# vovach777/llcomp

Hardware: AMD Instinct MI355X
Metric: encode+decode MPix/s on 4K RGB8, bit-exact (higher is better)
Workload: dtype int32

## Files before the change

### llcomp_amd/csrc/dec_rows_asm.hpp

```cpp
#pragma once
#include <cstdint>

namespace llcomp_mi {

#define LD_E0L "v32"
#define LD_E0H "v33"
#define LD_E0 "v[32:33]"
#define LD_E5L "v34"
#define LD_E5H "v35"
#define LD_E5 "v[34:35]"
#define LD_E6L "v36"
#define LD_E6H "v37"
#define LD_E6 "v[36:37]"
#define LD_E7L "v38"
#define LD_E7H "v39"
#define LD_E7 "v[38:39]"
#define LD_E1L "v40"
#define LD_E1H "v41"
#define LD_E1 "v[40:41]"
#define LD_E2L "v42"
#define LD_E2H "v43"
#define LD_E2 "v[42:43]"
#define LD_E3L "v44"
#define LD_E3H "v45"
#define LD_E3 "v[44:45]"
#define LD_E4L "v48"
#define LD_E4H "v49"
#define LD_E4 "v[48:49]"
#define LD_WINL "v46"
#define LD_WIN "v[46:47]"
#define LD_PROD "v50"
#define LD_R1 "v51"
#define LD_DIFF "v52"
#define LD_OFF "v52"
#define LD_EX "v32"
#define LD_W "v33"
#define LD_RUN "v40"
#define LD_NX "v41"
#define LD_T "v42"
#define LD_SX "s[56:57]"
#define LD_SA "s[58:59]"
#define LD_SW "s[60:61]"
#define LD_SP "s[62:63]"
#define LD_S5 "s[64:65]"
#define LD_SU "s[66:67]"
#define LD_SD "s[68:69]"
#define LD_S1L "s[68:69]"
#define LD_SM "s[70:71]"
#define LD_S1 "s70"
#define LD_S2 "s71"

#define LD_SPLIT(EL)                                                                                                       \
    "v_mul_u32_u24_sdwa " LD_PROD ", " EL ", %[range] dst_sel:DWORD dst_unused:UNUSED_PAD src0_sel:BYTE_1 src1_sel:DWORD\n\t" \
    "v_lshrrev_b32_e32 " LD_R1 ", 8, " LD_PROD "\n\t"                                                                      \
    "v_sub_u32_e32 %[range], %[range], " LD_R1 "\n\t"
#define LD_REFILL(N)                                         \
    "v_cmp_gt_u32_e32 vcc, %[c100], %[range]\n\t"            \
    "s_and_saveexec_b64 " LD_SW ", vcc\n\t"                  \
    "s_cbranch_execz .Lrf" N "_%=\n\t"                       \
    "v_lshlrev_b32_e32 %[range], 8, %[range]\n\t"            \
    "v_perm_b32 %[low], %[low], %[w32], %[sel]\n\t"          \
    "v_lshrrev_b32_e32 %[w32], 8, %[w32]\n"                   \
    ".Lrf" N "_%=:\n\t"                                      \
    "s_mov_b64 exec, " LD_SW "\n\t"
#define LD_REFILL_R1(N)                                           \
    "v_cmp_gt_u32_e32 vcc, %[c100], " LD_R1 "\n\t"                \
    "s_and_saveexec_b64 " LD_SW ", vcc\n\t"                       \
    "s_cbranch_execz .Lrf" N "_%=\n\t"                            \
    "v_and_b32_e32 %[range], 0xffffff00, " LD_PROD "\n\t"         \
    "v_perm_b32 %[low], %[low], %[w32], %[sel]\n\t"               \
    "v_lshrrev_b32_e32 %[w32], 8, %[w32]\n"                        \
    ".Lrf" N "_%=:\n\t"                                           \
    "s_mov_b64 exec, " LD_SW "\n\t"
#define LD_UNARY(EL, EH, OFS, N, SAVE)                                      \
    LD_SPLIT(EL)                                                            \
    "v_sub_co_u32_e32 %[low], vcc, %[low], %[range]\n\t"                    \
    "ds_write_b16_d16_hi %[bank], " EL " offset:" OFS "\n\t"                \
    "s_andn2_b64 exec, exec, vcc\n\t"                                       \
    SAVE                                                                    \
    "s_cbranch_execz .Lx_done_%=\n\t"                                       \
    "ds_write_b16_d16_hi %[bank], " EH " offset:" OFS "\n\t"                \
    "v_add_u32_e32 " LD_EX ", 1, " LD_EX "\n\t"                                     \
    "v_mov_b32_e32 %[range], " LD_R1 "\n\t"                                 \
    LD_REFILL_R1(N)
#define LD_FETCH_REST                                         \
    "v_lshrrev_b32_e32 " LD_E1L ", 16, %[w0]\n\t"             \
    "v_and_b32_e32 " LD_E2L ", 0xffff, %[w1]\n\t"             \
    "v_lshrrev_b32_e32 " LD_E3L ", 16, %[w1]\n\t"             \
    "v_and_b32_e32 " LD_E4L ", 0xffff, %[w2]\n\t"             \
    "ds_read_b64 " LD_E1 ", " LD_E1L "\n\t"                   \
    "ds_read_b64 " LD_E2 ", " LD_E2L "\n\t"                   \
    "ds_read_b64 " LD_E3 ", " LD_E3L "\n\t"                   \
    "ds_read_b64 " LD_E4 ", " LD_E4L "\n\t"                   \
    "v_lshrrev_b32_e32 " LD_E5L ", 16, %[w2]\n\t"             \
    "v_and_b32_e32 " LD_E6L ", 0xffff, %[w3]\n\t"             \
    "v_lshrrev_b32_e32 " LD_E7L ", 16, %[w3]\n\t"             \
    "ds_read_b64 " LD_E5 ", " LD_E5L "\n\t"                   \
    "ds_read_b64 " LD_E6 ", " LD_E6L "\n\t"                   \
    "ds_read_b64 " LD_E7 ", " LD_E7L "\n\t"

__device__ __forceinline__ void dec_rows_sample_asm(uint32_t& low, uint32_t& range, unsigned long long& win, uint32_t w0, uint32_t w1,
                                                    uint32_t w2, uint32_t w3, uint32_t bank, uint32_t& hot, uint32_t& value, uint32_t& w32) {
    asm volatile(
        "s_mov_b64 " LD_SX ", exec\n\t"
        "v_and_b32_e32 %[w32], 0xffffff, " LD_WINL "\n\t"
        "v_or_b32_e32 %[w32], 0x1000000, %[w32]\n\t"
        "v_and_b32_e32 " LD_OFF ", 0xffff, %[w0]\n\t"
        "ds_read_b64 " LD_E0 ", " LD_OFF "\n\t"
        "v_mov_b32_e32 %[value], 0\n\t"
        "s_cmp_lg_u32 %[hot], 0\n\t"
        "s_cbranch_scc0 .Lcold_%=\n\t"
        LD_FETCH_REST
        "s_waitcnt lgkmcnt(7)\n\t"
        "s_branch .Lzero_%=\n"
        ".Lcold_%=:\n\t"
        "s_waitcnt lgkmcnt(0)\n"
        ".Lzero_%=:\n\t"
        LD_SPLIT(LD_E0L)
        "v_sub_co_u32_e32 " LD_DIFF ", vcc, %[low], %[range]\n\t"
        "ds_write_b16_d16_hi %[bank], " LD_E0L "\n\t"
        "s_and_b64 " LD_SA ", exec, vcc\n\t"
        "s_andn2_b64 exec, exec, vcc\n\t"
        "s_cbranch_execz .Lz1_%=\n\t"
        "v_mov_b32_e32 %[low], " LD_DIFF "\n\t"
        "v_mov_b32_e32 %[range], " LD_R1 "\n\t"
        "ds_write_b16_d16_hi %[bank], " LD_E0H "\n"
        ".Lz1_%=:\n\t"
        "s_mov_b64 exec, " LD_SX "\n\t"
        LD_REFILL("0")
        "s_and_b64 exec, " LD_SA ", " LD_SA "\n\t"
        "s_cbranch_execz .Ldone_%=\n\t"
        "s_cmp_lg_u32 %[hot], 0\n\t"
        "s_cbranch_scc1 .Lhave_%=\n\t"
        LD_FETCH_REST
        ".Lhave_%=:\n\t"
        "v_mov_b32_e32 " LD_EX ", 0\n\t"
        "v_mov_b32_e32 " LD_W ", 1\n\t"
        "s_waitcnt lgkmcnt(0)\n\t"
        "s_mov_b64 " LD_SM ", 0\n\t"
        LD_UNARY(LD_E1L, LD_E1H, "2", "1", "s_mov_b64 " LD_S1L ", exec\n\t")
        LD_UNARY(LD_E2L, LD_E2H, "256", "2", "s_mov_b64 " LD_SM ", exec\n\t")
        LD_UNARY(LD_E3L, LD_E3H, "258", "3", "")
        "s_mov_b64 " LD_SU ", exec\n\t"
        ".p2align 6\n"
        ".Lu_%=:\n\t"
        "s_waitcnt lgkmcnt(0)\n\t"
        LD_SPLIT(LD_E4L)
// ... 73 lines not shown
        "v_lshlrev_b32_e32 " LD_W ", " LD_T ", " LD_W "\n\t"
        "v_or_b32_e32 " LD_W ", " LD_W ", " LD_RUN "\n"
        ".Lvalue_%=:\n\t"
        "s_mov_b64 exec, " LD_S5 "\n\t"
        "v_lshlrev_b32_e64 " LD_T ", " LD_EX ", 1\n\t"
        "v_add_u32_e32 " LD_T ", -1, " LD_T "\n\t"
        "v_xor_b32_e32 %[value], " LD_W ", " LD_T "\n\t"
        LD_SPLIT(LD_E7L)
        "v_sub_co_u32_e32 " LD_DIFF ", vcc, %[low], %[range]\n\t"
        "ds_write_b16_d16_hi %[bank], " LD_E7L " offset:770\n\t"
        "s_andn2_b64 exec, exec, vcc\n\t"
        "s_cbranch_execz .Lp7_%=\n\t"
        "v_mov_b32_e32 %[low], " LD_DIFF "\n\t"
        "v_mov_b32_e32 %[range], " LD_R1 "\n\t"
        "ds_write_b16_d16_hi %[bank], " LD_E7H " offset:770\n\t"
        "v_sub_u32_e32 %[value], 0, %[value]\n"
        ".Lp7_%=:\n\t"
        "s_mov_b64 exec, " LD_S5 "\n\t"
        LD_REFILL("7")
        ".Ldone_%=:\n\t"
        "s_mov_b64 exec, " LD_SX "\n\t"
        "v_ffbh_u32_e32 " LD_DIFF ", %[w32]\n\t"
        "v_add_u32_e32 " LD_DIFF ", -7, " LD_DIFF "\n\t"
        "v_lshrrev_b64 " LD_WIN ", " LD_DIFF ", " LD_WIN "\n\t"
        "s_bcnt1_i32_b64 " LD_S1 ", " LD_SA "\n\t"
        "s_bcnt1_i32_b64 " LD_S2 ", " LD_SX "\n\t"
        "s_lshl_b32 " LD_S1 ", " LD_S1 ", 1\n\t"
        "s_cmp_ge_u32 " LD_S1 ", " LD_S2 "\n\t"
        "s_cselect_b32 %[hot], 1, 0\n\t"
        "s_mov_b64 exec, " LD_SX "\n\t"
        : [low] "+v"(low), [range] "+v"(range), "+{v[46:47]}"(win), [hot] "+s"(hot), [value] "=&v"(value), [w32] "=&v"(w32)
        : [w0] "v"(w0), [w1] "v"(w1), [w2] "v"(w2), [w3] "v"(w3), [bank] "v"(bank), [c100] "s"(0x100u), [sel] "s"(0x06050400u),
          [sentv] "v"(0x80000000u)
        : "vcc", "scc", "memory", "v32", "v33", "v34", "v35", "v36", "v37", "v38", "v39", "v40", "v41", "v42", "v43", "v44", "v45",
          "v48", "v49", "v50", "v51", "v52", "s56", "s57", "s58", "s59", "s60", "s61", "s62", "s63", "s64", "s65", "s66",
          "s67", "s68", "s69", "s70", "s71");
}

}
```

### llcomp_amd/csrc/slice_kernels.hip

```cpp
#include <algorithm>

#include "device_common.hpp"
#include "kernels.hpp"

#ifndef LLMI_ASM_ENC
#define LLMI_ASM_ENC 1
#endif
#if LLMI_ASM_ENC
#include "enc_rows_asm.hpp"
#endif
#ifndef LLMI_ASM_DEC
#define LLMI_ASM_DEC 1
#endif
#if LLMI_ASM_DEC
#include "dec_rows_asm.hpp"
#endif

namespace llcomp_mi {

namespace {

#ifdef LLMI_CLOCK_PROBE
constexpr uint32_t kProbeSlots = 1u << 15;
__device__ unsigned long long g_probe[2][kProbeSlots][2];
// ... 116 lines not shown
    E.e2 = tab[slot_state<2>(bank)];
    E.e3 = tab[slot_state<3>(bank)];
    E.e4 = tab[slot_state<4>(bank)];
    E.e5 = tab[slot_state<5>(bank)];
    E.e6 = tab[slot_state<6>(bank)];
    E.e7 = tab[slot_state<7>(bank)];
}

__device__ __forceinline__ entry_t entry_at(const entry_t*, uint32_t nx) { return lds_entry(nx >> 16); }

__device__ __forceinline__ void publish_count(unsigned long long* counters, uint32_t which, uint32_t mine) {
    if (!counters) return;
    unsigned long long live = __ballot(mine != 0);
    if (live == 0) return;
    unsigned long long sum = 0;
    const unsigned long long all = __ballot(1);
    while (live) {
        const int lane = __builtin_ctzll(live);
        sum += uint32_t(__builtin_amdgcn_readlane(mine, lane));
        live &= live - 1;
    }
    if (threadIdx.x == uint32_t(__builtin_ctzll(all))) atomicAdd(counters + which, sum);
}

struct RangeEnc {
    uint32_t low;
    uint32_t range;
    uint32_t wp;
    uint32_t base;
    uint8_t* area;
    int32_t flushed;
    uint8_t* out;
    uint8_t* gout;
    uint32_t oofs;
    uint32_t ostep;
    int32_t cap;
    uint32_t shift;
    uint32_t carries;
};
constexpr int kStageBytes = 32;
constexpr int kStagePad = 16;
__device__ __forceinline__ int32_t enc_pos(const RangeEnc& e) { return e.flushed + int32_t(e.wp - e.base); }
__device__ __forceinline__ uint8_t* unit_byte(RangeEnc& e, uint32_t k) {
    return e.out + ((size_t(k >> 4) << (e.shift + 4)) + (k & 15));
}
__device__ __forceinline__ void enc_flush16(RangeEnc& e) {
// ... 136 lines not shown
                uint32_t nx;
                uint32_t bits = ((a << 1) | 1u) << (32 - ex);
                do {
                    nx = enc_step_msb(e, bits, cur);
                    cur = lds_entry(nx);
                } while (bits != 0x80000000u);
                put_state<6, INLDS>(bank, (nx - lds_address(tab)) >> 3);
            }
        }
        enc_once<7, INLDS>(e, bank, E, res < 0);
    }
}

__device__ __forceinline__ void enc_finish_and_count(RangeEnc& e, int32_t& n_bytes) {
    e.range = 0xFF; e.low += 0xFF; enc_renorm(e);
    e.range = 0xFF; enc_renorm(e);
    n_bytes = enc_pos(e);
    while (int32_t(e.wp - e.base) > 0) enc_flush16(e);
}

extern __shared__ __attribute__((aligned(32))) unsigned char dyn_lds[];
constexpr uint32_t kRowsEncTabOff = 0, kRowsEncStageOff = 1024, kRowsEncBankOff = 1024 + 16 + 32 * 64;
constexpr uint32_t kRowsEncLdsBytes = kRowsEncBankOff + 3 * 64 * 8;
[[maybe_unused]] __device__ __forceinline__ void enc_carry_back_flushed(RangeEnc& e) {
    if (e.flushed > 0 && e.flushed - 1 < e.cap) ++e.carries;
    for (int32_t k = e.flushed - 1; k >= 0; --k) {
        if (k >= e.cap) break;
        uint8_t* g = unit_byte(e, uint32_t(k));
        const uint32_t v = *g;
        *g = uint8_t(v + 1);
        if (v != 0xFF) break;
    }
}
template <bool LDSTAB>
__device__ __forceinline__ void clear_lds_states() {
    if constexpr (LDSTAB) {
        unsigned long long* t = reinterpret_cast<unsigned long long*>(dyn_lds);
        for (uint32_t i = threadIdx.x; i < uint32_t(kContexts); i += blockDim.x) t[i] = 0;
    }
}
template <int NCH, bool ROWS, typename SYM, bool LDSTAB = false, bool SNAP = false, bool SEG = false>
__global__ __launch_bounds__(64) void k_encode_slices(const Geometry g, const uint32_t lpw,
                                                      const SYM* __restrict__ sym, uint64_t* __restrict__ states,
                                                      uint8_t* __restrict__ scratch, uint32_t* __restrict__ slice_len,
                                                      uint64_t* __restrict__ group_sum, uint32_t* status, const uint64_t gpat,
                                                      unsigned long long* __restrict__ counters, const uint32_t seg_first = 0,
                                                      uint32_t* __restrict__ seg_state = nullptr) {
    static_assert(!(SNAP && (ROWS || LDSTAB)) && (SNAP || !SEG), "one kernel family at a time");
    constexpr bool ASM = (ROWS || SNAP) && LLMI_ASM_ENC != 0;
    entry_t* tab;
    uint8_t* stage;
    uint32_t* rowbank;
    if constexpr (ASM) {
        static_assert(kStagePad == 16 && kStageBytes == 32, "kRowsEncBankOff");
#ifdef LLMI_TEST_LDS_OFFSET
        __shared__ uint32_t s_displace[4];
        if (threadIdx.x < 4) reinterpret_cast<volatile uint32_t*>(s_displace)[threadIdx.x] = gpat != 0;
#endif
        tab = reinterpret_cast<entry_t*>(dyn_lds + kRowsEncTabOff);
        stage = dyn_lds + kRowsEncStageOff;
        rowbank = reinterpret_cast<uint32_t*>(dyn_lds + kRowsEncBankOff);
        if (uint32_t(uintptr_t((lds_u8_ptr)dyn_lds)) != 0) {
            if (threadIdx.x == 0) atomicOr(status, kStInternal);
            return;
        }
    } else {
        __shared__ entry_t s_tab[128];
        __shared__ __attribute__((aligned(32))) uint8_t s_stage[kStagePad + kStageBytes * 64];
        __shared__ uint32_t s_rowbank[ROWS ? kRowBankWords : 1];
        tab = s_tab;
        stage = s_stage;
// ... 46 lines not shown
        if constexpr (SEG) {
            if (seg_first >= total) return;
            i = seg_first;
            end = min(total, seg_first + kSnapMaxSamples);
            if (seg_first) {
                const uint4 a = *reinterpret_cast<const uint4*>(rec), b = *reinterpret_cast<const uint4*>(rec + 4);
                const uint4 s0 = *reinterpret_cast<const uint4*>(rec + 8), s1 = *reinterpret_cast<const uint4*>(rec + 12);
                e.low = a.x; e.range = a.y; e.wp = e.base + a.z; e.flushed = int32_t(a.w);
                e.carries = b.x; hot = b.y != 0;
                e.oofs += (uint32_t(e.flushed) >> 4) * e.ostep;
                uint32_t* const st = reinterpret_cast<uint32_t*>(e.area);
                st[0] = s0.x; st[1] = s0.y; st[2] = s0.z; st[3] = s0.w; st[4] = s1.x; st[5] = s1.y; st[6] = s1.z; st[7] = s1.w;
            }
        }
#if LLMI_ASM_ENC
        EncRowsExtra xs{0u, 0u, 0u};
        unsigned long long low_range = e.low | ((unsigned long long)e.range << 32);
#endif
        auto code = [&](int res, uint2 bk) {
#if LLMI_ASM_ENC
            enc_snap_sample_asm(low_range, e.wp, xs, bk.x, bk.y, res, e.base);
            if (__builtin_expect(xs.any_pend != 0, 0)) {
                xs.any_pend = 0;
                if (xs.pend) enc_carry_back_flushed(e);
                xs.pend = 0;
            }
#else
            Bank bank{{bk.x, bk.y}, nullptr};
            if (hot) enc_residual<true, false>(e, bank, tab, res); else enc_residual<false, false>(e, bank, tab, res);
            hot = __builtin_amdgcn_readfirstlane(2 * __popcll(__ballot(res != 0)) >= __popcll(__ballot(true)));
#endif
        };
        const uint32_t todo = end - i, todo0 = __builtin_amdgcn_readfirstlane(todo);
        const bool same = __builtin_amdgcn_ballot_w64(todo != todo0) == 0;
        const uint32_t n_bulk = i + (same ? todo0 & ~3u : 0);
        int r0 = load_res(i), r1 = load_res(i + 1), r2 = load_res(i + 2), r3 = load_res(i + 3);
        uint2 b0 = load_bank(i), b1 = load_bank(i + 1), b2 = load_bank(i + 2), b3 = load_bank(i + 3);
#define LLMI_SNAP_SAMPLE(R, B, AHEAD)                          \
        {                                                          \
            const int rc = int(consume_here(uint32_t(R)));        \
            uint2 bc = B;                                          \
            bc.x = consume_here(bc.x);                             \
            R = load_res(i + AHEAD);                               \
            B = load_bank(i + AHEAD);                              \
            if (e.wp >= e.base + 16) enc_flush16(e);               \
            code(rc, bc);                                          \
        }
// ... 13 lines not shown
            }
        }
#undef LLMI_SNAP_SAMPLE
#if LLMI_ASM_ENC
        e.low = uint32_t(low_range);
        e.range = uint32_t(low_range >> 32);
#endif
        if constexpr (SEG) {
            if (end < total) {
                const uint32_t* const st = reinterpret_cast<const uint32_t*>(e.area);
                *reinterpret_cast<uint4*>(rec) = make_uint4(e.low, e.range, e.wp - e.base, uint32_t(e.flushed));
                *reinterpret_cast<uint4*>(rec + 4) = make_uint4(e.carries, hot ? 1u : 0u, 0u, 0u);
                *reinterpret_cast<uint4*>(rec + 8) = make_uint4(st[0], st[1], st[2], st[3]);
                *reinterpret_cast<uint4*>(rec + 12) = make_uint4(st[4], st[5], st[6], st[7]);
                return;
            }
        }
    } else if constexpr (ROWS) {
        for (uint32_t k = 0; k < 6; ++k) rowbank[k * 64 + threadIdx.x] = 0;
        constexpr bool PX = sizeof(SYM) == 1;
        const char* gsym;
        uint32_t sofs, sstep;
        [[maybe_unused]] uint32_t n_dword = total;
        [[maybe_unused]] uint32_t psh = 0, msub = 0, my = 0, large = 0;
        [[maybe_unused]] int pl = 128, pL = 128;
        if constexpr (PX) {
            const uint32_t C = g.c;
            const unsigned long long tbase = ((unsigned long long)(r.frame) * g.h + r.y0) * g.w * C + (unsigned long long)(r.x0) * C;
            const unsigned long long wbase = (unsigned long long)uint32_t(__builtin_amdgcn_readfirstlane(uint32_t(tbase))) |
                                             ((unsigned long long)uint32_t(__builtin_amdgcn_readfirstlane(uint32_t(tbase >> 32))) << 32);
            gsym = reinterpret_cast<const char*>(sym) + wbase;
            sofs = uint32_t(tbase - wbase);
            sstep = C;
            const unsigned long long total_bytes = (unsigned long long)(g.frames) * g.h * g.w * C;
            n_dword = rows_px_dwords(tbase, total, C, total_bytes);
            psh = 8 * r.ch;
            msub = C >= 3 && (r.ch == 0 || r.ch == 2) ? ~0u : 0u;
            my = C >= 3 && r.ch == 1 ? ~0u : 0u;
            large = (g.flags & kGeoSmallModel) ? 0u : ~0u;
            asm volatile("" : "+v"(psh), "+v"(msub), "+v"(my));
        } else {
            const uint32_t grp = __builtin_amdgcn_readfirstlane(id >> g.lane_shift);
            gsym = reinterpret_cast<const char*>(sym + ((size_t(grp) * g.slice_samples) << g.lane_shift));
            sofs = (id & ((1u << g.lane_shift) - 1)) * uint32_t(sizeof(SYM));
            sstep = uint32_t(sizeof(SYM)) << g.lane_shift;
        }
        asm volatile("" : "+v"(sstep));
        auto load_sym = [&](uint32_t ofs) -> uint32_t {
            if constexpr (PX) {
                uint32_t w;
                __builtin_memcpy(&w, gsym + ofs, 4);
                return w;
            } else {
                return *reinterpret_cast<const SYM*>(gsym + ofs);
            }
        };
        auto load_at = [&](uint32_t ofs, uint32_t k) -> uint32_t {
            if constexpr (PX) {
                if (k >= n_dword) {
                    const uint8_t* p = reinterpret_cast<const uint8_t*>(gsym + ofs);
                    uint32_t w = p[0];
                    if (g.c > 1) w |= uint32_t(p[1]) << 8;
                    if (g.c > 2) w |= uint32_t(p[2]) << 16;
                    if (g.c > 3) w |= uint32_t(p[3]) << 24;
                    return w;
                }
            }
            return load_sym(ofs);
        };
        uint32_t s0 = load_at(sofs, 0);
        sofs += sstep;
        uint32_t s1 = total > 1 ? load_at(sofs, 1) : 0;
        sofs += sstep;
        uint32_t bank_base = uint32_t(uintptr_t((lds_u8_ptr) reinterpret_cast<uint8_t*>(rowbank))) + threadIdx.x * 4;
        asm volatile("" : "+v"(bank_base));
#if LLMI_ASM_ENC
        EncRowsExtra xs{0u, 0u, 0u};
        unsigned long long low_range = e.low | ((unsigned long long)e.range << 32);
#endif
        auto code = [&](uint32_t sy, uint32_t i) {
            uint32_t bofs;
            int res;
            if constexpr (PX) {
                const uint32_t G = (sy >> 8) & 0xFF;
                const int sum = int(sy & 0xFF) + int((sy >> 16) & 0xFF) - 2 * int(G);
                const int t = (sum + int((uint32_t(sum) >> 31) * 3u)) >> 2;
                const int v = int(__builtin_amdgcn_ubfe(sy, psh, 8)) - int(G & msub) + (t & int(my));
                const int dq = (pL - pl) & int(i >= 2 ? large : 0u);
                const int sg = dq >> 31;
                const uint32_t aq = uint32_t((dq ^ sg) - sg);
                bofs = ((aq + 511u) & 0x200u) + ((aq + 508u) & 0x200u);
                res = ((v - pl) ^ sg) - sg;
                pL = pl;
                pl = v;
            } else if constexpr (sizeof(SYM) == 2) {
                bofs = (sy >> 3) & 0x600u;
                res = int(sy << 20) >> 20;
            } else {
                bofs = (((sy & 0xFFFF) * 109u) >> 7) & 0x600u;
                res = int(sy) >> 16;
            }
#if LLMI_ASM_ENC
            enc_rows_sample_asm(low_range, e.wp, xs, bank_base + bofs, res, e.base);
            if (__builtin_expect(xs.any_pend != 0, 0)) {
                xs.any_pend = 0;
                if (xs.pend) enc_carry_back_flushed(e);
                xs.pend = 0;
            }
#else
            uint32_t* bp = reinterpret_cast<uint32_t*>(reinterpret_cast<uint8_t*>(rowbank) + threadIdx.x * 4 + bofs);
            Bank bank{{bp[0], bp[64]}, reinterpret_cast<uint8_t*>(bp)};
            if (hot) enc_residual<true, true>(e, bank, tab, res); else enc_residual<false, true>(e, bank, tab, res);
            hot = __builtin_amdgcn_readfirstlane(2 * __popcll(__ballot(res != 0)) >= __popcll(__ballot(true)));
#endif
        };
        const uint32_t total0 = __builtin_amdgcn_readfirstlane(total);
        const bool same = __builtin_amdgcn_ballot_w64(total != total0) == 0;
        const uint32_t tail = PX ? rows_px_tail(g.c) : 2u;
        const uint32_t n_bulk = same && total0 > tail ? total0 - tail : 0;
        uint32_t i = 0;
        for (; i < n_bulk; ++i) {
            s0 = consume_here(s0);
            const uint32_t s2 = load_sym(sofs);
            sofs += sstep;
            if (e.wp >= e.base + 16) enc_flush16(e);
            code(s0, i);
            s0 = s1;
            s1 = s2;
        }
        for (; i < total; ++i) {
            s0 = consume_here(s0);
            const uint32_t s2 = i + 2 < total ? load_at(sofs, i + 2) : 0;
            sofs += sstep;
            if (e.wp >= e.base + 16) enc_flush16(e);
            code(s0, i);
            s0 = s1;
            s1 = s2;
        }
#if LLMI_ASM_ENC
        e.low = uint32_t(low_range);
        e.range = uint32_t(low_range >> 32);
#endif
    } else {
        uint64_t* banks;
        uint32_t bsh;
        if constexpr (LDSTAB) {
            banks = reinterpret_cast<uint64_t*>(dyn_lds);
            bsh = 0;
        } else {
            banks = states + ((size_t(id >> g.lane_shift) * kContexts) << g.lane_shift) + (id & ((1u << g.lane_shift) - 1));
            bsh = g.lane_shift;
        }
        uint32_t fk = 0;
        auto fetch = [&]() -> uint32_t { return p0[size_t(fk++) * GW]; };
        uint32_t s0 = fetch();
        uint32_t s1 = total > 1 ? fetch() : 0;
        uint64_t b0 = bank_fresh<LDSTAB>(banks[size_t(s0 & 0xFFFF) << bsh], gpat);
        for (uint32_t i = 0; i < total; ++i) {
            const uint32_t s2 = i + 2 < total ? fetch() : 0;
            const uint32_t ctx0 = s0 & 0xFFFF, ctx1 = s1 & 0xFFFF;
            const int res = int(s0) >> 16;
// ... 201 lines not shown
    if (ex > 0) {
        w += w + uint32_t(!dec_once<5, CHECKED, INLDS>(d, bank, E));
        if (ex > 1) {
            entry_t cur = E.e6;
            uint32_t nx;
            uint32_t limit = ones + 1;
            asm volatile("" : "+v"(limit));
            do {
                nx = dec_step_acc<CHECKED>(d, prob_of(cur), cur, w);
                cur = entry_at(tab, nx);
            } while (w < limit);
            dec_put_state<6, INLDS>(bank, nx);
        }
    }
    uint32_t v = w ^ ones;
    if (dec_once<7, CHECKED, INLDS>(d, bank, E)) v = 0u - v;
    out = v;
    return true;
}

template <bool INLDS>
__device__ __forceinline__ bool dec_sample(RangeDec& d, Bank& bank, const entry_t* tab, uint32_t& hot, bool replay_always,
                                           uint32_t& v) {
    const uint32_t s_low = d.low, s_range = d.range, s_b0 = bank.w[0], s_b1 = bank.w[1], s_b2 = bank.w[2], s_b3 = bank.w[3];
    const unsigned long long s_win = d.win;
    bool ok;
#if LLMI_ASM_DEC
    if constexpr (INLDS) {
        uint32_t left;
        dec_rows_sample_asm(d.low, d.range, d.win, bank.w[0], bank.w[1], bank.w[2], bank.w[3], lds_address(bank.lds), hot, v, left);
        ok = left != 0;
    } else
#endif
    {
        ok = hot ? dec_residual<true, false, INLDS>(d, bank, tab, v) : dec_residual<false, false, INLDS>(d, bank, tab, v);
        hot = 2 * __popcll(__ballot(v != 0)) >= __popcll(__ballot(true));
    }
    const bool ran_dry = (INLDS && LLMI_ASM_DEC != 0) ? false : d.win == 0;
    if (__builtin_expect(!ok || ran_dry || replay_always, 0)) {
        ++d.replays;
        d.low = s_low; d.range = s_range; d.win = s_win;
        bank.w[0] = s_b0; bank.w[1] = s_b1;
        if constexpr (INLDS) {
            bank.w[2] = s_b2; bank.w[3] = s_b3;
            reinterpret_cast<uint32_t*>(bank.lds)[0] = s_b0;
            reinterpret_cast<uint32_t*>(bank.lds)[64] = s_b1;
            reinterpret_cast<uint32_t*>(bank.lds)[128] = s_b2;
            reinterpret_cast<uint32_t*>(bank.lds)[192] = s_b3;
        }
        ok = dec_residual<false, true, INLDS>(d, bank, tab, v);
    }
    return ok;
}

constexpr uint32_t bank_cache_lds_bytes(int log2_entries) { return log2_entries ? (64u * 9u) << log2_entries : 0u; }
template <int NCH, bool ROWS, bool LDSTAB = false, int CACHE = 0>
__global__ __launch_bounds__(64) void k_decode_slices(const Geometry g, const uint32_t lpw_and_flags,
                                                      const uint8_t* __restrict__ units,
                                                      const uint32_t* __restrict__ slice_len,
                                                      uint64_t* __restrict__ states, int16_t* __restrict__ rec,
                                                      uint32_t* status, const uint64_t gpat,
                                                      unsigned long long* __restrict__ counters) {
    __shared__ entry_t tab[128];
    __shared__ uint32_t rowbank[ROWS ? kWideBankWords : 1];
    __shared__ int8_t quant_lut[ROWS ? 1 : 512];
    if constexpr (!ROWS) {
        for (uint32_t i = threadIdx.x; i < 256; i += blockDim.x) {
            quant_lut[i] = int8_t(quant11(int(i) - 128));
            quant_lut[256 + i] = int8_t(quant5(int(i) - 128));
        }
    }
    static_assert(CACHE == 0 || (!ROWS && !LDSTAB && NCH != 0), "the bank cache belongs to the 2-D kernels with tables in HBM");
    static_assert(CACHE == 0 || ((kContexts - 1) >> CACHE) < 0xFF, "bank cache: a context's tag would alias the empty marker");
    __shared__ uint32_t wave_sums[CACHE != 0 ? 2 : 1];
    clear_lds_states<LDSTAB>();
    if constexpr (CACHE != 0) {
        uint32_t* tg = reinterpret_cast<uint32_t*>(dyn_lds + (512u << CACHE));
        for (uint32_t i = threadIdx.x; i < (16u << CACHE); i += blockDim.x) tg[i] = 0xFFFFFFFFu;
        if (threadIdx.x < 2) wave_sums[threadIdx.x] = 0;
    }
    load_table(tab);
    const uint32_t lpw = lpw_and_flags & 0xFF;
    const bool replay_always = (lpw_and_flags >> 8) & 1;
    const bool small_model = (g.flags & kGeoSmallModel) != 0;
    const uint32_t id = blockIdx.x * lpw + threadIdx.x;
    if (threadIdx.x >= lpw || id >= g.n_slices) return;
    const SliceRect r = slice_rect(g, id);
    RangeDec d;
    const uint32_t len = min(slice_len[id], g.slice_cap - 16);
    const uint32_t grp = __builtin_amdgcn_readfirstlane(id >> g.lane_shift);
    const uint32_t lane_in_group = id & ((1u << g.lane_shift) - 1);
    dec_open(d, reinterpret_cast<const uint32_t*>(units) + ((size_t(grp) * (g.slice_cap >> 2)) << g.lane_shift), lane_in_group,
             g.lane_shift, len);

    int16_t* p0 = rec + lane_order_index(g, id, 0);
    const ptrdiff_t GW = ptrdiff_t(1) << g.lane_shift;
    int16_t* const gbase = rec + ((size_t(grp) * g.slice_samples) << g.lane_shift);
    uint32_t hot = 0;
    LLMI_PROBE_START();

    if constexpr (ROWS) {
        for (uint32_t k = 0; k < 12; ++k) rowbank[k * 64 + threadIdx.x] = lds_address(tab) * 0x00010001u;
        int l[NCH], L[NCH];
#pragma unroll
        for (int k = 0; k < NCH; ++k) l[k] = L[k] = 128;
        int held_val = 0;
        uint32_t held_ofs = lane_in_group * 2, next_ofs = held_ofs, step_ofs = 2u << g.lane_shift;
        uint32_t large = small_model ? 0u : ~0u, first = ~0u;
        asm volatile("" : "+v"(large), "+v"(first), "+v"(step_ofs));
        uint8_t* const bank0 = reinterpret_cast<uint8_t*>(rowbank) + threadIdx.x * 4;
        bool bad = false;
        auto pixel = [&]() {
#pragma unroll
            for (int k = 0; k < NCH; ++k) {
                if (window_low(d)) dec_append(d);
                asm volatile("global_store_short %0, %1, %2" : : "v"(held_ofs), "v"(held_val), "s"(gbase) : "memory");
                const int lv = l[k];
                const int dq = (L[k] - lv) & int(large);
                int sg = dq >> 31;
                asm volatile("" : "+v"(sg));
                const uint32_t aq = uint32_t((dq ^ sg) - sg);
                uint32_t o1 = ((aq + 0x7FFFFFFFu) >> 21) & 0x400u, o2 = ((aq + 0x7FFFFFFCu) >> 21) & 0x400u;
                asm volatile("" : "+v"(o1), "+v"(o2));
                uint32_t* bp = reinterpret_cast<uint32_t*>(bank0 + (o1 + o2));
                Bank bank{{bp[0], bp[64], bp[128], bp[192]}, reinterpret_cast<uint8_t*>(bp)};
                uint32_t v = 0;
                if (!dec_sample<true>(d, bank, tab, hot, replay_always, v)) bad = true;
                v = (v ^ uint32_t(sg)) - uint32_t(sg);
                const int val = int(int16_t(uint32_t(lv) + v));
                held_val = val;
                held_ofs = next_ofs;
                next_ofs += step_ofs;
                L[k] = lv ^ ((lv ^ val) & int(first));
                l[k] = val;
            }
            first = 0;
        };
        const uint32_t sw0 = __builtin_amdgcn_readfirstlane(r.sw);
        const uint32_t n_bulk = __builtin_amdgcn_ballot_w64(r.sw != sw0) == 0 ? sw0 : 0;
        uint32_t x = 0;
        for (; x < n_bulk; ++x) pixel();
        for (; x < r.sw; ++x) pixel();
        if (bad) atomicOr(status, kStBadExponent);
        asm volatile("global_store_short %0, %1, %2" : : "v"(held_ofs), "v"(held_val), "s"(gbase) : "memory");
        publish_count(counters, kCtrDecReplays, d.replays);
    } else {
        uint64_t* banks;
        uint32_t bsh;
        if constexpr (LDSTAB) {
            banks = reinterpret_cast<uint64_t*>(dyn_lds);
            bsh = 0;
        } else {
            banks = states + ((size_t(id >> g.lane_shift) * kContexts) << g.lane_shift) + (id & ((1u << g.lane_shift) - 1));
            bsh = g.lane_shift;
        }
        if constexpr (NCH == 0) {
            const uint32_t nch = g.nch;
            const ptrdiff_t px_step = ptrdiff_t(nch) * GW, up = ptrdiff_t(r.sw) * px_step;
            for (uint32_t y = 0; y < r.sh; ++y) {
                for (uint32_t x = 0; x < r.sw; ++x) {
                    for (uint32_t k = 0; k < nch; ++k) {
                        int16_t* q = p0 + ptrdiff_t(y) * up + ptrdiff_t(x) * px_step + ptrdiff_t(k) * GW;
                        if (window_low(d)) dec_append(d);
                        const Hood n = apply_borders(x > 0 ? q[-px_step] : 0, x > 1 ? q[-2 * px_step] : 0, y > 0 ? q[-up] : 0,
                                                     (y > 0 && x > 0) ? q[-up - px_step] : 0, (y > 0 && x + 1 < r.sw) ? q[-up + px_step] : 0,
                                                     y > 1 ? q[-2 * up] : 0, x, y, r.sw);
                        int ctx = context_hash(n, small_model);
// ... 211 lines not shown
                                 uint32_t* d_status, unsigned long long* d_counters, uint32_t seg_first, uint32_t* d_seg_state,
                                 hipStream_t stream) {
    if (!coder_in_segments(g) || !d_seg_state) return hipErrorInvalidValue;
    const uint32_t blocks = (g.n_slices + g.lpw - 1) / g.lpw;
    k_encode_slices<0, false, uint32_t, false, true, true><<<dim3(blocks), dim3(64), LLMI_ASM_ENC ? kRowsEncLdsBytes : 0, stream>>>(
        g, g.lpw, static_cast<const uint32_t*>(d_res), d_banks, d_scratch, d_slice_len, nullptr, d_status, 0, d_counters, seg_first, d_seg_state);
    return hipGetLastError();
}

uint64_t state_generation_tag(uint32_t generation) {
    uint64_t t = 0;
    for (int i = 0; i < 8; ++i) t |= uint64_t((generation >> i) & 1u) << (8 * i + 7);
    return t;
}

hipError_t launch_encode_slices(const Geometry& g, const void* d_sym, uint64_t* d_states, uint32_t generation, uint8_t* d_scratch,
                                uint32_t* d_slice_len, uint64_t* d_group_off, uint32_t* d_status, unsigned long long* d_counters,
                                hipStream_t stream) {
    const uint64_t gpat = slices_need_state_tables(g) ? state_generation_tag(generation) : 0;
    const uint32_t lpw = g.lpw;
    const uint32_t blocks = (g.n_slices + lpw - 1) / lpw;
    uint64_t* const d_group_sum = encoder_writes_group_sums(g) ? d_group_off : nullptr;
    if (rows_encoder_reads_pixels(g)) {
        k_encode_slices<1, true, uint8_t><<<dim3(blocks), dim3(64), LLMI_ASM_ENC ? kRowsEncLdsBytes : 0, stream>>>(
            g, lpw, static_cast<const uint8_t*>(d_sym), d_states, d_scratch, d_slice_len, d_group_sum, d_status, gpat, d_counters);
        return hipGetLastError();
    }
    if (model_is_fused(g)) {
        k_encode_slices<1, true, uint16_t><<<dim3(blocks), dim3(64), LLMI_ASM_ENC ? kRowsEncLdsBytes : 0, stream>>>(
            g, lpw, static_cast<const uint16_t*>(d_sym), d_states, d_scratch, d_slice_len, d_group_sum, d_status, gpat, d_counters);
        return hipGetLastError();
    }
    if (g.flags & kGeoSnapshot) {
        k_encode_slices<0, false, uint32_t, false, true><<<dim3(blocks), dim3(64), LLMI_ASM_ENC ? kRowsEncLdsBytes : 0, stream>>>(
            g, lpw, static_cast<const uint32_t*>(d_sym), d_states, d_scratch, d_slice_len, d_group_sum, d_status, 0, d_counters);
        return hipGetLastError();
    }
    const bool lds = states_in_lds(g);
    LLMI_DISPATCH_SLICE(g.nch, rows_mode(g), lds, {
        auto kernel = k_encode_slices<C, R, uint32_t, T>;
        if (T) {
            const hipError_t e = allow_big_lds(kernel);
            if (e != hipSuccess) return e;
        }
        kernel<<<dim3(blocks), dim3(64), T ? kLdsTableBytes : (R && LLMI_ASM_ENC ? kRowsEncLdsBytes : 0), stream>>>(
            g, lpw, static_cast<const uint32_t*>(d_sym), d_states, d_scratch, d_slice_len, d_group_sum, d_status, gpat, d_counters, 0u, nullptr);
    });
    return hipGetLastError();
// ... 3 lines not shown
                                uint64_t* d_states, uint32_t generation, int16_t* d_rec, uint32_t* d_status, unsigned long long* d_counters,
                                bool bank_cache, hipStream_t stream) {
    const uint64_t gpat = slices_need_state_tables(g) ? state_generation_tag(generation) : 0;
    const uint32_t lpw = g.lpw;
    const uint32_t blocks = (g.n_slices + lpw - 1) / lpw;
    const uint32_t arg = lpw | ((g.flags & kGeoForceReplay) ? 0x100u : 0u);
    const bool lds = states_in_lds(g);
    if (bank_cache_log2(g) == kBankCacheLog2 && bank_cache) {
#define LLMI_DECODE_CACHED(NCHV)                                                                                          \
    k_decode_slices<NCHV, false, false, kBankCacheLog2><<<dim3(blocks), dim3(64), bank_cache_lds_bytes(kBankCacheLog2), stream>>>( \
        g, arg, d_units, d_slice_len, d_states, d_rec, d_status, gpat, d_counters)
        switch (g.nch) {
            case 1: LLMI_DECODE_CACHED(1); break;
            case 2: LLMI_DECODE_CACHED(2); break;
            case 3: LLMI_DECODE_CACHED(3); break;
            case 4: LLMI_DECODE_CACHED(4); break;
            default: return hipErrorInvalidValue;
        }
#undef LLMI_DECODE_CACHED
        return hipGetLastError();
    }
    LLMI_DISPATCH_SLICE(g.nch, rows_mode(g), lds, {
        auto kernel = k_decode_slices<C, R, T>;
        if (T) {
            const hipError_t e = allow_big_lds(kernel);
            if (e != hipSuccess) return e;
        }
        kernel<<<dim3(blocks), dim3(64), T ? kLdsTableBytes : 0, stream>>>(g, arg, d_units, d_slice_len, d_states,
                                                                          d_rec, d_status, gpat, d_counters);
    });
    return hipGetLastError();
}

}
```

Measured before the change: 29430.

## Specialize rows encode/decode on model size, peel first samples, unroll hot loops

Turns the small/large context-model choice into a template parameter so the per-sample masking and sign-fold arithmetic disappear from the small-model path. The first sample or two are peeled, which removes the per-iteration `first` and `i>=2` masks, and the bulk loops are unrolled by two. The decode asm now takes separate input and output state, so the replay path no longer keeps saved copies, and it uses a cndmask in place of a branchy move. Launch bounds are raised to request 8 waves per EU on the row kernels. The cost is more kernel instantiations, and the tighter register budget from the new launch bounds risks spills.

```diff
diff --git a/llcomp_amd/csrc/dec_rows_asm.hpp b/llcomp_amd/csrc/dec_rows_asm.hpp
--- a/llcomp_amd/csrc/dec_rows_asm.hpp
+++ b/llcomp_amd/csrc/dec_rows_asm.hpp
@@ -27,8 +27,6 @@
 #define LD_E4L "v48"
 #define LD_E4H "v49"
 #define LD_E4 "v[48:49]"
-#define LD_WINL "v46"
-#define LD_WIN "v[46:47]"
 #define LD_PROD "v50"
 #define LD_R1 "v51"
 #define LD_DIFF "v52"
@@ -54,6 +52,10 @@
     "v_mul_u32_u24_sdwa " LD_PROD ", " EL ", %[range] dst_sel:DWORD dst_unused:UNUSED_PAD src0_sel:BYTE_1 src1_sel:DWORD\n\t" \
     "v_lshrrev_b32_e32 " LD_R1 ", 8, " LD_PROD "\n\t"                                                                      \
     "v_sub_u32_e32 %[range], %[range], " LD_R1 "\n\t"
+#define LD_SPLIT_IN(EL)                                                                                                       \
+    "v_mul_u32_u24_sdwa " LD_PROD ", " EL ", %[range_in] dst_sel:DWORD dst_unused:UNUSED_PAD src0_sel:BYTE_1 src1_sel:DWORD\n\t" \
+    "v_lshrrev_b32_e32 " LD_R1 ", 8, " LD_PROD "\n\t"                                                                      \
+    "v_sub_u32_e32 %[range], %[range_in], " LD_R1 "\n\t"
 #define LD_REFILL(N)                                         \
     "v_cmp_gt_u32_e32 vcc, %[c100], %[range]\n\t"            \
     "s_and_saveexec_b64 " LD_SW ", vcc\n\t"                  \
@@ -99,11 +101,12 @@
     "ds_read_b64 " LD_E6 ", " LD_E6L "\n\t"                   \
     "ds_read_b64 " LD_E7 ", " LD_E7L "\n\t"
 
-__device__ __forceinline__ void dec_rows_sample_asm(uint32_t& low, uint32_t& range, unsigned long long& win, uint32_t w0, uint32_t w1,
-                                                    uint32_t w2, uint32_t w3, uint32_t bank, uint32_t& hot, uint32_t& value, uint32_t& w32) {
+__device__ __forceinline__ void dec_rows_sample_asm(uint32_t low_in, uint32_t range_in, unsigned long long win_in, uint32_t& low,
+                                                    uint32_t& range, unsigned long long& win, uint32_t w0, uint32_t w1, uint32_t w2,
+                                                    uint32_t w3, uint32_t bank, uint32_t& hot, uint32_t& value, uint32_t& w32) {
     asm volatile(
         "s_mov_b64 " LD_SX ", exec\n\t"
-        "v_and_b32_e32 %[w32], 0xffffff, " LD_WINL "\n\t"
+        "v_and_b32_e32 %[w32], 0xffffff, %[winl_in]\n\t"
         "v_or_b32_e32 %[w32], 0x1000000, %[w32]\n\t"
         "v_and_b32_e32 " LD_OFF ", 0xffff, %[w0]\n\t"
         "ds_read_b64 " LD_E0 ", " LD_OFF "\n\t"
@@ -116,13 +119,13 @@
         ".Lcold_%=:\n\t"
         "s_waitcnt lgkmcnt(0)\n"
         ".Lzero_%=:\n\t"
-        LD_SPLIT(LD_E0L)
-        "v_sub_co_u32_e32 " LD_DIFF ", vcc, %[low], %[range]\n\t"
+        LD_SPLIT_IN(LD_E0L)
+        "v_sub_co_u32_e32 %[low], vcc, %[low_in], %[range]\n\t"
         "ds_write_b16_d16_hi %[bank], " LD_E0L "\n\t"
         "s_and_b64 " LD_SA ", exec, vcc\n\t"
+        "v_cndmask_b32_e32 %[low], %[low], %[low_in], vcc\n\t"
         "s_andn2_b64 exec, exec, vcc\n\t"
         "s_cbranch_execz .Lz1_%=\n\t"
-        "v_mov_b32_e32 %[low], " LD_DIFF "\n\t"
         "v_mov_b32_e32 %[range], " LD_R1 "\n\t"
         "ds_write_b16_d16_hi %[bank], " LD_E0H "\n"
         ".Lz1_%=:\n\t"
@@ -242,15 +245,15 @@
         "s_mov_b64 exec, " LD_SX "\n\t"
         "v_ffbh_u32_e32 " LD_DIFF ", %[w32]\n\t"
         "v_add_u32_e32 " LD_DIFF ", -7, " LD_DIFF "\n\t"
-        "v_lshrrev_b64 " LD_WIN ", " LD_DIFF ", " LD_WIN "\n\t"
+        "v_lshrrev_b64 %[win], " LD_DIFF ", %[win_in]\n\t"
         "s_bcnt1_i32_b64 " LD_S1 ", " LD_SA "\n\t"
         "s_bcnt1_i32_b64 " LD_S2 ", " LD_SX "\n\t"
         "s_lshl_b32 " LD_S1 ", " LD_S1 ", 1\n\t"
         "s_cmp_ge_u32 " LD_S1 ", " LD_S2 "\n\t"
         "s_cselect_b32 %[hot], 1, 0\n\t"
         "s_mov_b64 exec, " LD_SX "\n\t"
-        : [low] "+v"(low), [range] "+v"(range), "+{v[46:47]}"(win), [hot] "+s"(hot), [value] "=&v"(value), [w32] "=&v"(w32)
-        : [w0] "v"(w0), [w1] "v"(w1), [w2] "v"(w2), [w3] "v"(w3), [bank] "v"(bank), [c100] "s"(0x100u), [sel] "s"(0x06050400u),
+        : [low] "=&v"(low), [range] "=&v"(range), [win] "=&v"(win), [hot] "+s"(hot), [value] "=&v"(value), [w32] "=&v"(w32)
+        : [low_in] "v"(low_in), [range_in] "v"(range_in), [win_in] "v"(win_in), [winl_in] "v"(uint32_t(win_in)), [w0] "v"(w0), [w1] "v"(w1), [w2] "v"(w2), [w3] "v"(w3), [bank] "v"(bank), [c100] "s"(0x100u), [sel] "s"(0x06050400u),
           [sentv] "v"(0x80000000u)
         : "vcc", "scc", "memory", "v32", "v33", "v34", "v35", "v36", "v37", "v38", "v39", "v40", "v41", "v42", "v43", "v44", "v45",
           "v48", "v49", "v50", "v51", "v52", "s56", "s57", "s58", "s59", "s60", "s61", "s62", "s63", "s64", "s65", "s66",
diff --git a/llcomp_amd/csrc/slice_kernels.hip b/llcomp_amd/csrc/slice_kernels.hip
--- a/llcomp_amd/csrc/slice_kernels.hip
+++ b/llcomp_amd/csrc/slice_kernels.hip
@@ -1,4 +1,5 @@
 #include <algorithm>
+#include <type_traits>
 
 #include "device_common.hpp"
 #include "kernels.hpp"
@@ -162,6 +163,10 @@
     }
     if (threadIdx.x == uint32_t(__builtin_ctzll(all))) atomicAdd(counters + which, sum);
 }
+
+constexpr int kModelSmall = 0;
+constexpr int kModelLarge = 1;
+constexpr std::integral_constant<int, kModelSmall> no_model{};
 
 struct RangeEnc {
     uint32_t low;
@@ -344,11 +349,11 @@
 extern __shared__ __attribute__((aligned(32))) unsigned char dyn_lds[];
 constexpr uint32_t kRowsEncTabOff = 0, kRowsEncStageOff = 1024, kRowsEncBankOff = 1024 + 16 + 32 * 64;
 constexpr uint32_t kRowsEncLdsBytes = kRowsEncBankOff + 3 * 64 * 8;
-[[maybe_unused]] __device__ __forceinline__ void enc_carry_back_flushed(RangeEnc& e) {
+[[maybe_unused]] __device__ __forceinline__ void enc_carry_back_flushed(RangeEnc& e, uint8_t* out) {
     if (e.flushed > 0 && e.flushed - 1 < e.cap) ++e.carries;
     for (int32_t k = e.flushed - 1; k >= 0; --k) {
         if (k >= e.cap) break;
-        uint8_t* g = unit_byte(e, uint32_t(k));
+        uint8_t* g = out + ((size_t(uint32_t(k) >> 4) << (e.shift + 4)) + (uint32_t(k) & 15));
         const uint32_t v = *g;
         *g = uint8_t(v + 1);
         if (v != 0xFF) break;
@@ -361,14 +366,15 @@
         for (uint32_t i = threadIdx.x; i < uint32_t(kContexts); i += blockDim.x) t[i] = 0;
     }
 }
-template <int NCH, bool ROWS, typename SYM, bool LDSTAB = false, bool SNAP = false, bool SEG = false>
-__global__ __launch_bounds__(64) void k_encode_slices(const Geometry g, const uint32_t lpw,
+template <int NCH, bool ROWS, typename SYM, bool LDSTAB = false, bool SNAP = false, bool SEG = false, bool SMALL = false>
+__global__ __launch_bounds__(64, ROWS ? 8 : 1) void k_encode_slices(const Geometry g, const uint32_t lpw,
                                                       const SYM* __restrict__ sym, uint64_t* __restrict__ states,
                                                       uint8_t* __restrict__ scratch, uint32_t* __restrict__ slice_len,
                                                       uint64_t* __restrict__ group_sum, uint32_t* status, const uint64_t gpat,
                                                       unsigned long long* __restrict__ counters, const uint32_t seg_first = 0,
                                                       uint32_t* __restrict__ seg_state = nullptr) {
     static_assert(!(SNAP && (ROWS || LDSTAB)) && (SNAP || !SEG), "one kernel family at a time");
+    static_assert(!SMALL || (ROWS && sizeof(SYM) == 1), "the model is a template flag only where the kernel forms the contexts");
     constexpr bool ASM = (ROWS || SNAP) && LLMI_ASM_ENC != 0;
     entry_t* tab;
     uint8_t* stage;
@@ -461,7 +467,7 @@
             enc_snap_sample_asm(low_range, e.wp, xs, bk.x, bk.y, res, e.base);
             if (__builtin_expect(xs.any_pend != 0, 0)) {
                 xs.any_pend = 0;
-                if (xs.pend) enc_carry_back_flushed(e);
+                if (xs.pend) enc_carry_back_flushed(e, e.out);
                 xs.pend = 0;
             }
 #else
@@ -521,7 +527,7 @@
         const char* gsym;
         uint32_t sofs, sstep;
         [[maybe_unused]] uint32_t n_dword = total;
-        [[maybe_unused]] uint32_t psh = 0, msub = 0, my = 0, large = 0;
+        [[maybe_unused]] uint32_t psh = 0, msub = 0, my = 0;
         [[maybe_unused]] int pl = 128, pL = 128;
         if constexpr (PX) {
             const uint32_t C = g.c;
@@ -536,7 +542,6 @@
             psh = 8 * r.ch;
             msub = C >= 3 && (r.ch == 0 || r.ch == 2) ? ~0u : 0u;
             my = C >= 3 && r.ch == 1 ? ~0u : 0u;
-            large = (g.flags & kGeoSmallModel) ? 0u : ~0u;
             asm volatile("" : "+v"(psh), "+v"(msub), "+v"(my));
         } else {
             const uint32_t grp = __builtin_amdgcn_readfirstlane(id >> g.lane_shift);
@@ -577,19 +582,41 @@
         EncRowsExtra xs{0u, 0u, 0u};
         unsigned long long low_range = e.low | ((unsigned long long)e.range << 32);
 #endif
-        auto code = [&](uint32_t sy, uint32_t i) {
-            uint32_t bofs;
-            int res;
+        auto front = [&](uint32_t sy) -> uint32_t {
+            uint32_t t = sy;
             if constexpr (PX) {
                 const uint32_t G = (sy >> 8) & 0xFF;
                 const int sum = int(sy & 0xFF) + int((sy >> 16) & 0xFF) - 2 * int(G);
-                const int t = (sum + int((uint32_t(sum) >> 31) * 3u)) >> 2;
-                const int v = int(__builtin_amdgcn_ubfe(sy, psh, 8)) - int(G & msub) + (t & int(my));
-                const int dq = (pL - pl) & int(i >= 2 ? large : 0u);
-                const int sg = dq >> 31;
-                const uint32_t aq = uint32_t((dq ^ sg) - sg);
-                bofs = ((aq + 511u) & 0x200u) + ((aq + 508u) & 0x200u);
-                res = ((v - pl) ^ sg) - sg;
+                const int q = (sum + int((uint32_t(sum) >> 31) * 3u)) >> 2;
+                t = uint32_t(int(__builtin_amdgcn_ubfe(sy, psh, 8)) - int(G & msub) + (q & int(my)));
+            }
+            asm volatile("" : "+v"(t) : : "memory");
+            return t;
+        };
+        struct Ctx {
+            uint32_t bofs;
+            int sg;
+        };
+        auto context = [&](auto model) -> Ctx {
+            constexpr int MODEL = decltype(model)::value;
+            Ctx c{0u, 0};
+            if constexpr (PX && MODEL != kModelSmall) {
+                const int dq = pL - pl;
+                c.sg = dq >> 31;
+                asm volatile("" : "+v"(c.sg));
+                const uint32_t aq = uint32_t((dq ^ c.sg) - c.sg);
+                c.bofs = ((aq + 511u) & 0x200u) + ((aq + 508u) & 0x200u);
+                asm volatile("" : "+v"(c.bofs));
+            }
+            return c;
+        };
+        auto code = [&](uint32_t sy, Ctx c, auto model) {
+            constexpr int MODEL = decltype(model)::value;
+            uint32_t bofs = c.bofs;
+            int res;
+            if constexpr (PX) {
+                const int v = int(sy);
+                res = MODEL == kModelSmall ? v - pl : ((v - pl) ^ c.sg) - c.sg;
                 pL = pl;
                 pl = v;
             } else if constexpr (sizeof(SYM) == 2) {
@@ -603,7 +630,7 @@
             enc_rows_sample_asm(low_range, e.wp, xs, bank_base + bofs, res, e.base);
             if (__builtin_expect(xs.any_pend != 0, 0)) {
                 xs.any_pend = 0;
-                if (xs.pend) enc_carry_back_flushed(e);
+                if (xs.pend) enc_carry_back_flushed(e, e.gout + (size_t(id & ((1u << g.lane_shift) - 1)) << 4));
                 xs.pend = 0;
             }
 #else
@@ -617,25 +644,44 @@
         const bool same = __builtin_amdgcn_ballot_w64(total != total0) == 0;
         const uint32_t tail = PX ? rows_px_tail(g.c) : 2u;
         const uint32_t n_bulk = same && total0 > tail ? total0 - tail : 0;
-        uint32_t i = 0;
-        for (; i < n_bulk; ++i) {
+        auto sample_tested = [&](uint32_t i, auto model) {
             s0 = consume_here(s0);
-            const uint32_t s2 = load_sym(sofs);
-            sofs += sstep;
-            if (e.wp >= e.base + 16) enc_flush16(e);
-            code(s0, i);
-            s0 = s1;
-            s1 = s2;
-        }
-        for (; i < total; ++i) {
-            s0 = consume_here(s0);
+            const Ctx c0 = context(model);
+            const uint32_t t0 = front(s0);
             const uint32_t s2 = i + 2 < total ? load_at(sofs, i + 2) : 0;
             sofs += sstep;
             if (e.wp >= e.base + 16) enc_flush16(e);
-            code(s0, i);
+            code(t0, c0, model);
             s0 = s1;
             s1 = s2;
-        }
+        };
+        auto bulk = [&](uint32_t& i, auto model) {
+            for (; i + 1 < n_bulk; i += 2) {
+                s0 = consume_here(s0);
+                const Ctx c0 = context(model);
+                const uint32_t t0 = front(s0);
+                s0 = load_sym(sofs);
+                sofs += sstep;
+                if (e.wp >= e.base + 16) enc_flush16(e);
+                code(t0, c0, model);
+                s1 = consume_here(s1);
+                const Ctx c1 = context(model);
+                const uint32_t t1 = front(s1);
+                s1 = load_sym(sofs);
+                sofs += sstep;
+                if (e.wp >= e.base + 16) enc_flush16(e);
+                code(t1, c1, model);
+            }
+            for (; i < total; ++i) sample_tested(i, model);
+        };
+        sample_tested(0, no_model);
+        if (total > 1) sample_tested(1, no_model);
+#if LLMI_ASM_ENC
+        xs.hot = __builtin_amdgcn_readfirstlane(xs.hot);
+        xs.any_pend = 0;
+#endif
+        uint32_t i = 2;
+        bulk(i, std::integral_constant<int, SMALL ? kModelSmall : kModelLarge>{});
 #if LLMI_ASM_ENC
         e.low = uint32_t(low_range);
         e.range = uint32_t(low_range >> 32);
@@ -883,40 +929,57 @@
 template <bool INLDS>
 __device__ __forceinline__ bool dec_sample(RangeDec& d, Bank& bank, const entry_t* tab, uint32_t& hot, bool replay_always,
                                            uint32_t& v) {
-    const uint32_t s_low = d.low, s_range = d.range, s_b0 = bank.w[0], s_b1 = bank.w[1], s_b2 = bank.w[2], s_b3 = bank.w[3];
-    const unsigned long long s_win = d.win;
-    bool ok;
 #if LLMI_ASM_DEC
     if constexpr (INLDS) {
-        uint32_t left;
-        dec_rows_sample_asm(d.low, d.range, d.win, bank.w[0], bank.w[1], bank.w[2], bank.w[3], lds_address(bank.lds), hot, v, left);
-        ok = left != 0;
+        uint32_t low, range, left;
+        unsigned long long win;
+        dec_rows_sample_asm(d.low, d.range, d.win, low, range, win, bank.w[0], bank.w[1], bank.w[2], bank.w[3], lds_address(bank.lds), hot, v,
+                            left);
+        if (__builtin_expect(left == 0 || replay_always, 0)) {
+            ++d.replays;
+            reinterpret_cast<uint32_t*>(bank.lds)[0] = bank.w[0];
+            reinterpret_cast<uint32_t*>(bank.lds)[64] = bank.w[1];
+            reinterpret_cast<uint32_t*>(bank.lds)[128] = bank.w[2];
+            reinterpret_cast<uint32_t*>(bank.lds)[192] = bank.w[3];
+            asm("v_mov_b32_e32 %0, %3\n\tv_mov_b32_e32 %1, %4\n\tv_mov_b64_e32 %2, %5"
+                : "+v"(low), "+v"(range), "+v"(win)
+                : "v"(d.low), "v"(d.range), "v"(d.win));
+            d.low = low;
+            d.range = range;
+            d.win = win;
+            return dec_residual<false, true, true>(d, bank, tab, v);
+        }
+        d.low = low;
+        d.range = range;
+        d.win = win;
+        return true;
     } else
 #endif
     {
-        ok = hot ? dec_residual<true, false, INLDS>(d, bank, tab, v) : dec_residual<false, false, INLDS>(d, bank, tab, v);
+        const uint32_t s_low = d.low, s_range = d.range, s_b0 = bank.w[0], s_b1 = bank.w[1], s_b2 = bank.w[2], s_b3 = bank.w[3];
+        const unsigned long long s_win = d.win;
+        bool ok = hot ? dec_residual<true, false, INLDS>(d, bank, tab, v) : dec_residual<false, false, INLDS>(d, bank, tab, v);
         hot = 2 * __popcll(__ballot(v != 0)) >= __popcll(__ballot(true));
-    }
-    const bool ran_dry = (INLDS && LLMI_ASM_DEC != 0) ? false : d.win == 0;
-    if (__builtin_expect(!ok || ran_dry || replay_always, 0)) {
-        ++d.replays;
-        d.low = s_low; d.range = s_range; d.win = s_win;
-        bank.w[0] = s_b0; bank.w[1] = s_b1;
-        if constexpr (INLDS) {
-            bank.w[2] = s_b2; bank.w[3] = s_b3;
-            reinterpret_cast<uint32_t*>(bank.lds)[0] = s_b0;
-            reinterpret_cast<uint32_t*>(bank.lds)[64] = s_b1;
-            reinterpret_cast<uint32_t*>(bank.lds)[128] = s_b2;
-            reinterpret_cast<uint32_t*>(bank.lds)[192] = s_b3;
-        }
-        ok = dec_residual<false, true, INLDS>(d, bank, tab, v);
-    }
-    return ok;
+        if (__builtin_expect(!ok || d.win == 0 || replay_always, 0)) {
+            ++d.replays;
+            d.low = s_low; d.range = s_range; d.win = s_win;
+            bank.w[0] = s_b0; bank.w[1] = s_b1;
+            if constexpr (INLDS) {
+                bank.w[2] = s_b2; bank.w[3] = s_b3;
+                reinterpret_cast<uint32_t*>(bank.lds)[0] = s_b0;
+                reinterpret_cast<uint32_t*>(bank.lds)[64] = s_b1;
+                reinterpret_cast<uint32_t*>(bank.lds)[128] = s_b2;
+                reinterpret_cast<uint32_t*>(bank.lds)[192] = s_b3;
+            }
+            ok = dec_residual<false, true, INLDS>(d, bank, tab, v);
+        }
+        return ok;
+    }
 }
 
 constexpr uint32_t bank_cache_lds_bytes(int log2_entries) { return log2_entries ? (64u * 9u) << log2_entries : 0u; }
-template <int NCH, bool ROWS, bool LDSTAB = false, int CACHE = 0>
-__global__ __launch_bounds__(64) void k_decode_slices(const Geometry g, const uint32_t lpw_and_flags,
+template <int NCH, bool ROWS, bool LDSTAB = false, int CACHE = 0, bool SMALL = false>
+__global__ __launch_bounds__(64, ROWS && NCH == 1 ? 8 : 1) void k_decode_slices(const Geometry g, const uint32_t lpw_and_flags,
                                                       const uint8_t* __restrict__ units,
                                                       const uint32_t* __restrict__ slice_len,
                                                       uint64_t* __restrict__ states, int16_t* __restrict__ rec,
@@ -932,6 +995,7 @@
         }
     }
     static_assert(CACHE == 0 || (!ROWS && !LDSTAB && NCH != 0), "the bank cache belongs to the 2-D kernels with tables in HBM");
+    static_assert(!SMALL || ROWS, "the model is a template flag of the 1-row-slice kernels only");
     static_assert(CACHE == 0 || ((kContexts - 1) >> CACHE) < 0xFF, "bank cache: a context's tag would alias the empty marker");
     __shared__ uint32_t wave_sums[CACHE != 0 ? 2 : 1];
     clear_lds_states<LDSTAB>();
@@ -943,7 +1007,7 @@
     load_table(tab);
     const uint32_t lpw = lpw_and_flags & 0xFF;
     const bool replay_always = (lpw_and_flags >> 8) & 1;
-    const bool small_model = (g.flags & kGeoSmallModel) != 0;
+    [[maybe_unused]] const bool small_model = (g.flags & kGeoSmallModel) != 0;
     const uint32_t id = blockIdx.x * lpw + threadIdx.x;
     if (threadIdx.x >= lpw || id >= g.n_slices) return;
     const SliceRect r = slice_rect(g, id);
@@ -966,44 +1030,58 @@
 #pragma unroll
         for (int k = 0; k < NCH; ++k) l[k] = L[k] = 128;
         int held_val = 0;
-        uint32_t held_ofs = lane_in_group * 2, next_ofs = held_ofs, step_ofs = 2u << g.lane_shift;
-        uint32_t large = small_model ? 0u : ~0u, first = ~0u;
-        asm volatile("" : "+v"(large), "+v"(first), "+v"(step_ofs));
+        uint32_t store_ofs = lane_in_group * 2, step_ofs = 2u << g.lane_shift;
+        asm volatile("" : "+v"(step_ofs));
         uint8_t* const bank0 = reinterpret_cast<uint8_t*>(rowbank) + threadIdx.x * 4;
         bool bad = false;
-        auto pixel = [&]() {
+        auto pixel = [&](auto model, auto start) {
+            constexpr int MODEL = decltype(model)::value;
+            constexpr bool START = decltype(start)::value;
 #pragma unroll
             for (int k = 0; k < NCH; ++k) {
                 if (window_low(d)) dec_append(d);
-                asm volatile("global_store_short %0, %1, %2" : : "v"(held_ofs), "v"(held_val), "s"(gbase) : "memory");
+                if (!(START && k == 0)) {
+                    asm volatile("global_store_short %0, %1, %2" : : "v"(store_ofs), "v"(held_val), "s"(gbase) : "memory");
+                    store_ofs += step_ofs;
+                }
                 const int lv = l[k];
-                const int dq = (L[k] - lv) & int(large);
-                int sg = dq >> 31;
-                asm volatile("" : "+v"(sg));
-                const uint32_t aq = uint32_t((dq ^ sg) - sg);
-                uint32_t o1 = ((aq + 0x7FFFFFFFu) >> 21) & 0x400u, o2 = ((aq + 0x7FFFFFFCu) >> 21) & 0x400u;
-                asm volatile("" : "+v"(o1), "+v"(o2));
-                uint32_t* bp = reinterpret_cast<uint32_t*>(bank0 + (o1 + o2));
+                uint32_t sg = 0, bofs = 0;
+                if constexpr (MODEL != kModelSmall) {
+                    const int dq = L[k] - lv;
+                    sg = uint32_t(dq >> 31);
+                    asm volatile("" : "+v"(sg));
+                    const uint32_t aq = (uint32_t(dq) ^ sg) - sg;
+                    uint32_t o1 = ((aq + 0x7FFFFFFFu) >> 21) & 0x400u, o2 = ((aq + 0x7FFFFFFCu) >> 21) & 0x400u;
+                    asm volatile("" : "+v"(o1), "+v"(o2));
+                    bofs = o1 + o2;
+                }
+                uint32_t* bp = reinterpret_cast<uint32_t*>(bank0 + bofs);
                 Bank bank{{bp[0], bp[64], bp[128], bp[192]}, reinterpret_cast<uint8_t*>(bp)};
                 uint32_t v = 0;
                 if (!dec_sample<true>(d, bank, tab, hot, replay_always, v)) bad = true;
-                v = (v ^ uint32_t(sg)) - uint32_t(sg);
+                if constexpr (MODEL != kModelSmall) v = (v ^ sg) - sg;
                 const int val = int(int16_t(uint32_t(lv) + v));
                 held_val = val;
-                held_ofs = next_ofs;
-                next_ofs += step_ofs;
-                L[k] = lv ^ ((lv ^ val) & int(first));
+                L[k] = START ? val : lv;
                 l[k] = val;
             }
-            first = 0;
         };
         const uint32_t sw0 = __builtin_amdgcn_readfirstlane(r.sw);
         const uint32_t n_bulk = __builtin_amdgcn_ballot_w64(r.sw != sw0) == 0 ? sw0 : 0;
-        uint32_t x = 0;
-        for (; x < n_bulk; ++x) pixel();
-        for (; x < r.sw; ++x) pixel();
+        uint32_t x = 1;
+        pixel(no_model, std::true_type{});
+        constexpr std::integral_constant<int, SMALL ? kModelSmall : kModelLarge> model{};
+        if constexpr (NCH == 1) {
+            for (; x + 1 < n_bulk; x += 2) {
+                pixel(model, std::false_type{});
+                pixel(model, std::false_type{});
+            }
+        } else {
+            for (; x < n_bulk; ++x) pixel(model, std::false_type{});
+        }
+        for (; x < r.sw; ++x) pixel(model, std::false_type{});
         if (bad) atomicOr(status, kStBadExponent);
-        asm volatile("global_store_short %0, %1, %2" : : "v"(held_ofs), "v"(held_val), "s"(gbase) : "memory");
+        asm volatile("global_store_short %0, %1, %2" : : "v"(store_ofs), "v"(held_val), "s"(gbase) : "memory");
         publish_count(counters, kCtrDecReplays, d.replays);
     } else {
         uint64_t* banks;
@@ -1261,8 +1339,9 @@
     const uint32_t blocks = (g.n_slices + lpw - 1) / lpw;
     uint64_t* const d_group_sum = encoder_writes_group_sums(g) ? d_group_off : nullptr;
     if (rows_encoder_reads_pixels(g)) {
-        k_encode_slices<1, true, uint8_t><<<dim3(blocks), dim3(64), LLMI_ASM_ENC ? kRowsEncLdsBytes : 0, stream>>>(
-            g, lpw, static_cast<const uint8_t*>(d_sym), d_states, d_scratch, d_slice_len, d_group_sum, d_status, gpat, d_counters);
+        auto kernel = (g.flags & kGeoSmallModel) ? k_encode_slices<1, true, uint8_t, false, false, false, true> : k_encode_slices<1, true, uint8_t>;
+        kernel<<<dim3(blocks), dim3(64), LLMI_ASM_ENC ? kRowsEncLdsBytes : 0, stream>>>(
+            g, lpw, static_cast<const uint8_t*>(d_sym), d_states, d_scratch, d_slice_len, d_group_sum, d_status, gpat, d_counters, 0u, nullptr);
         return hipGetLastError();
     }
     if (model_is_fused(g)) {
@@ -1312,6 +1391,9 @@
     }
     LLMI_DISPATCH_SLICE(g.nch, rows_mode(g), lds, {
         auto kernel = k_decode_slices<C, R, T>;
+        if constexpr (R) {
+            if (g.flags & kGeoSmallModel) kernel = k_decode_slices<C, R, T, 0, true>;
+        }
         if (T) {
             const hipError_t e = allow_big_lds(kernel);
             if (e != hipSuccess) return e;
```

Result: faster. 29820 (median of 6 runs) (+1.3%).
